# turboderp-org/exllamav2

Measured on NVIDIA H100. Metric: decode tokens/sec (bs=1) Llama2-7B EXL2-4.0bpw, higher is better.
Workload: dtype fp16 (int2-8 weights, fp32 accumulate)

## Files before the change

### exllamav2_b200/csrc/gemv_i8.cu

```cuda
#include <string.h>

#include <algorithm>
#include <map>
#include <mutex>
#include <string>
#include <vector>

#include "gemv_i8.cuh"

namespace exl2b {

constexpr int I8_MAX_WARPS = 16;
constexpr int I8_MAX_CTAS = 320;

struct I8Mat {
    const uint8_t* packed;
    const void* wtab;
    const half* bias;
    half* c;
    half* c_perm;
    const uint16_t* out_invperm;
    int N, blk_base, clear;
};

constexpr uint32_t DF_FLUSH = 1, DF_BLOCK_DONE = 2, DF_GPTQ = 4;
constexpr int I8_BARS = 8;
constexpr int I8_LWIN = 2 * I8_BARS;

struct I8Params {
    I8Mat mat[I8_MAX_MATS];
    const uint4* plan_desc;
    const uint32_t* plan_first;
    const uint32_t* plan_cta;
    const uint32_t* plan_red;
    int num_mats, K, KS;
    const uint16_t* perm;
    const half* x;
    const half* x2;
    const half* norm_w;
    float norm_eps;
    int mode, x_permuted;
    int norm_permuted;
    int l2_prefetch;
    int arena;
    int srow;
    int busy_ctas;
    unsigned int* slot_cnt;
    unsigned long long* dbg;
    int dbg_cta;
    unsigned long long* dbg_rec;
};

struct I8Smem {
    uint32_t act, asum, ascale, emit, scl, lst, total;
};
__host__ __device__ inline I8Smem i8_smem_map(int warps, int arena, int KS, int srow) {
    auto up = [](uint32_t x) { return (x + 15u) & ~15u; };
    I8Smem m;
    m.act = up((uint32_t)warps * (uint32_t)arena);
    m.asum = up(m.act + (uint32_t)KS * 64u);
    m.ascale = up(m.asum + (uint32_t)KS * 4u);
    m.emit = up(m.ascale + (uint32_t)(KS / 4 + 1) * 4u);
    m.scl = up(m.emit + (uint32_t)warps * 256u);
    m.lst = up(m.scl + (uint32_t)(warps * I8_BARS * srow));
    m.total = up(m.lst + (uint32_t)(warps * I8_LWIN * 16));
    return m;
}

template <int BITS>
__device__ __forceinline__ void consume_slab(uint32_t wb, uint32_t xs, int lane, int (&am)[4], int (&ae)[2]) {
    constexpr int Pm = plane_main(BITS), Pe = plane_extra(BITS);
    if constexpr (BITS == 4) {
        const uint4 w4 = lds128(wb + lane * 16);
#pragma unroll
        for (int hf = 0; hf < 2; ++hf) {
            const uint4 xh = lds128(xs + hf * 16), xl = lds128(xs + 32 + hf * 16);
            const uint32_t wa = hf ? w4.z : w4.x, wc = hf ? w4.w : w4.y;
            const uint32_t lo0 = wa & 0x0f0f0f0fu, hi0 = wa & 0xf0f0f0f0u, lo1 = wc & 0x0f0f0f0fu, hi1 = wc & 0xf0f0f0f0u;
            am[0] = dp4a_us(lo0, xh.x, am[0]);
            am[1] = dp4a_uu(lo0, xl.x, am[1]);
            am[2] = dp4a_us(hi0, xh.y, am[2]);
            am[3] = dp4a_uu(hi0, xl.y, am[3]);
            am[0] = dp4a_us(lo1, xh.z, am[0]);
            am[1] = dp4a_uu(lo1, xl.z, am[1]);
            am[2] = dp4a_us(hi1, xh.w, am[2]);
            am[3] = dp4a_uu(hi1, xl.w, am[3]);
        }
        return;
    }
    uint32_t XH[8], XL[8];
    {
        const uint4 h0 = lds128(xs), h1 = lds128(xs + 16), l0 = lds128(xs + 32), l1 = lds128(xs + 48);
        XH[0] = h0.x; XH[1] = h0.y; XH[2] = h0.z; XH[3] = h0.w; XH[4] = h1.x; XH[5] = h1.y; XH[6] = h1.z; XH[7] = h1.w;
        XL[0] = l0.x; XL[1] = l0.y; XL[2] = l0.z; XL[3] = l0.w; XL[4] = l1.x; XL[5] = l1.y; XL[6] = l1.z; XL[7] = l1.w;
    }
    if constexpr (Pm == 4) {
        const uint4 w4 = lds128(wb + lane * 16);
        const uint32_t W[4] = {w4.x, w4.y, w4.z, w4.w};
#pragma unroll
        for (int j = 0; j < 4; ++j) {
            const uint32_t lo = W[j] & 0x0f0f0f0fu, hi = W[j] & 0xf0f0f0f0u;
            am[0] = dp4a_us(lo, XH[2 * j], am[0]);
            am[1] = dp4a_uu(lo, XL[2 * j], am[1]);
            am[2] = dp4a_us(hi, XH[2 * j + 1], am[2]);
            am[3] = dp4a_uu(hi, XL[2 * j + 1], am[3]);
        }
    } else if constexpr (Pm == 8) {
        const uint4 a4 = lds128(wb + lane * 16), b4 = lds128(wb + 512 + lane * 16);
        const uint32_t W[8] = {a4.x, a4.y, a4.z, a4.w, b4.x, b4.y, b4.z, b4.w};
#pragma unroll
        for (int w = 0; w < 8; ++w) {
            am[0] = dp4a_us(W[w], XH[w], am[0]);
            am[1] = dp4a_uu(W[w], XL[w], am[1]);
        }
    } else {
        const uint2 w2 = lds64(wb + lane * 8);
        const uint32_t W[2] = {w2.x, w2.y};
#pragma unroll
        for (int w = 0; w < 2; ++w)
#pragma unroll
            for (int i = 0; i < 4; ++i) {
                const uint32_t t = (W[w] >> (2 * i)) & 0x03030303u;
                am[0] = dp4a_us(t, XH[4 * w + i], am[0]);
                am[1] = dp4a_uu(t, XL[4 * w + i], am[1]);
            }
    }
    if constexpr (Pe == 1) {
        const uint32_t w = lds32(wb + 128 * Pm + lane * 4);
#pragma unroll
        for (int i = 0; i < 8; ++i) {
            const uint32_t t = (w >> i) & 0x01010101u;
            ae[0] = dp4a_us(t, XH[i], ae[0]);
            ae[1] = dp4a_uu(t, XL[i], ae[1]);
        }
    } else if constexpr (Pe == 2) {
        const uint2 w2 = lds64(wb + 128 * Pm + lane * 8);
        const uint32_t W[2] = {w2.x, w2.y};
#pragma unroll
        for (int w = 0; w < 2; ++w)
#pragma unroll
            for (int i = 0; i < 4; ++i) {
                const uint32_t t = (W[w] >> (2 * i)) & 0x03030303u;
                ae[0] = dp4a_us(t, XH[4 * w + i], ae[0]);
                ae[1] = dp4a_uu(t, XL[4 * w + i], ae[1]);
            }
    }
}

template <int BITS>
__device__ __forceinline__ int consume_stage(uint32_t slot, int n, uint32_t xs, uint32_t asum, int lane, int (&am)[4], int (&ae)[2]) {
    constexpr uint32_t bb = 128 * BITS;
    int S = 0;
    if constexpr (BITS == 4) {
        uint4 w4 = lds128(slot + lane * 16);
#pragma unroll 1
        for (int s = 0; s < n; ++s) {
            const uint4 wn = lds128(slot + (s + 1 < n ? s + 1 : s) * bb + lane * 16);
            const uint32_t x = xs + s * 64;
#pragma unroll
            for (int hf = 0; hf < 2; ++hf) {
                const uint4 xh = lds128(x + hf * 16), xl = lds128(x + 32 + hf * 16);
                const uint32_t wa = hf ? w4.z : w4.x, wc = hf ? w4.w : w4.y;
                const uint32_t lo0 = wa & 0x0f0f0f0fu, hi0 = wa & 0xf0f0f0f0u, lo1 = wc & 0x0f0f0f0fu, hi1 = wc & 0xf0f0f0f0u;
                am[0] = dp4a_us(lo0, xh.x, am[0]);
                am[1] = dp4a_uu(lo0, xl.x, am[1]);
                am[2] = dp4a_us(hi0, xh.y, am[2]);
                am[3] = dp4a_uu(hi0, xl.y, am[3]);
                am[0] = dp4a_us(lo1, xh.z, am[0]);
                am[1] = dp4a_uu(lo1, xl.z, am[1]);
                am[2] = dp4a_us(hi1, xh.w, am[2]);
                am[3] = dp4a_uu(hi1, xl.w, am[3]);
            }
            S += (int)lds32(asum + s * 4);
            w4 = wn;
        }
        return S;
    }
#pragma unroll 1
    for (int s = 0; s < n; ++s) {
        consume_slab<BITS>(slot + s * bb, xs + s * 64, lane, am, ae);
        S += (int)lds32(asum + s * 4);
    }
    return S;
}

struct I8OutPre {
    uint32_t add;
    uint32_t kp;
};
__device__ __forceinline__ int mat_of_block(const I8Params& P, int blk) {
    int mi = 0;
#pragma unroll
    for (int i = 1; i < I8_MAX_MATS; ++i)
        if (i < P.num_mats && blk >= P.mat[i].blk_base) mi = i;
    return mi;
}
__device__ __forceinline__ I8OutPre out_pre(const I8Params& P, int blk, int lane) {
    const I8Mat& m = P.mat[mat_of_block(P, blk)];
    const int n = (blk - m.blk_base) * 32 + lane;
    I8OutPre r = {0u, (uint32_t)n};
    if (n < m.N) {
        if (m.bias) r.add = __ldg(reinterpret_cast<const unsigned short*>(m.bias) + n);
        if (!m.clear) r.add |= (uint32_t)__ldcg(reinterpret_cast<const unsigned short*>(m.c) + n) << 16;
        if (m.c_perm && m.out_invperm) r.kp = __ldg(m.out_invperm + n);
    }
    return r;
}
__device__ __forceinline__ void finalize_block(const I8Params& P, int blk, int lane, const I8OutPre& pre, float v) {
    const I8Mat& m = P.mat[mat_of_block(P, blk)];
    const int n = (blk - m.blk_base) * 32 + lane;
    if (n < m.N) {
        v += __half2float(__ushort_as_half((unsigned short)(pre.add & 0xffffu)));
        v += __half2float(__ushort_as_half((unsigned short)(pre.add >> 16)));
        const half h = __float2half_rn(v);
        m.c[n] = h;
        if (m.c_perm) m.c_perm[pre.kp] = h;
    }
}

__device__ __forceinline__ half silu_h(half x) {
    const half e = hexp(__hneg(x));
    const half r = hrcp(__hadd(__float2half(1.0f), e));
    return __hmul(x, r);
}
__device__ __forceinline__ half2 silu_h2(half2 x) {
    const half2 e = h2exp(__hneg2(x));
    const half2 r = h2rcp(__hadd2(__float2half2_rn(1.0f), e));
    return __hmul2(x, r);
}
__device__ __forceinline__ half gelu_h(half x) {
    float xf = __half2float(x);
    const float t = 0.797884560803f * (xf + 0.044715f * xf * xf * xf);
    float th;
    asm("tanh.approx.f32 %0, %1;" : "=f"(th) : "f"(t));
    xf = 0.5f * xf * (1.0 + th);
    return __float2half_rn(xf);
}


template <int I8_WARPS>
__global__ void __launch_bounds__(I8_WARPS * 32, 2) gemv_i8_kernel(const __grid_constant__ I8Params P) {
    constexpr int I8_THREADS = I8_WARPS * 32;
    extern __shared__ __align__(128) uint8_t smem[];
    __shared__ uint64_t bars[I8_WARPS * I8_BARS];
    __shared__ float s_red[I8_WARPS];

    const int tid = threadIdx.x, warp = tid >> 5, lane = tid & 31;
    const int KS = P.KS;
    EXL2B_STAMP(P, 0);
    if (P.dbg_rec && tid == 0 && blockIdx.x < 160) P.dbg_rec[blockIdx.x * 4] = globaltimer();
    if (tid < I8_WARPS * I8_BARS) mbar_init(smem_addr(&bars[tid]), 1);
    mbar_fence_init();
    __syncthreads();
    griddep_launch_dependents();

    if ((int)blockIdx.x >= P.busy_ctas) {
        if (tid == 0) slot_hold(P.slot_cnt, P.busy_ctas);
        return;
    }

    const uint32_t cinfo = __ldg(P.plan_cta + blockIdx.x);
    const int blk0 = (int)(cinfo & 0xffffu), nb = (int)(cinfo >> 16);
    const uint32_t fw0 = __ldg(P.plan_first + blockIdx.x * I8_WARPS + warp), fw1 = __ldg(P.plan_first + blockIdx.x * I8_WARPS + warp + 1);
    const uint32_t f0 = fw0 & 0x3ffffffu, f1 = fw1 & 0x3ffffffu;
    const int nst = (int)(f1 - f0), n_pre = (int)(fw0 >> 26);
    const uint4* const list = P.plan_desc + f0;

    const I8Smem sm = i8_smem_map(I8_WARPS, P.arena, KS, P.srow);
    uint8_t* const act_g = smem + sm.act;
    int* const asum_s = reinterpret_cast<int*>(smem + sm.asum);
    float* const ascale_s = reinterpret_cast<float*>(smem + sm.ascale);
    float* const emit_base = reinterpret_cast<float*>(smem + sm.emit);
    uint32_t sbase;
    asm volatile("mov.u32 %0, %1;" : "=r"(sbase) : "r"(smem_addr(smem)));
    const uint32_t ring = sbase + (uint32_t)warp * (uint32_t)P.arena;
    const uint32_t act = sbase + sm.act, asum = sbase + sm.asum, ascale = sbase + sm.ascale;
    const uint32_t sring = sbase + sm.scl + (uint32_t)(warp * I8_BARS * P.srow), lwin = sbase + sm.lst + (uint32_t)(warp * I8_LWIN * 16);
    uint32_t bar0;
    asm volatile("mov.u32 %0, %1;" : "=r"(bar0) : "r"(smem_addr(&bars[warp * I8_BARS])));

    auto issue_stages = [&](int s0, int cnt, uint4 d) {
        if (lane < cnt) {
            const int s = s0 + lane;
            const uint32_t mi = (d.z >> 22) & 3u;
            const uint8_t* pk = mi == 0 ? P.mat[0].packed : (mi == 1 ? P.mat[1].packed : P.mat[2].packed);
            const uint8_t* wt = reinterpret_cast<const uint8_t*>(mi == 0 ? P.mat[0].wtab : (mi == 1 ? P.mat[1].wtab : P.mat[2].wtab));
            const uint32_t bytes = ((d.z >> 24) & 0xffu) << 7;
            const uint32_t esz = (d.z & (DF_GPTQ << 18)) ? 4u : 2u;
            const uint32_t sbytes = (d.z & (DF_FLUSH << 18)) ? 32u * esz : 0u;
            const bool lnext = s + I8_BARS < nst;
            const uint32_t slot = (uint32_t)s & (I8_BARS - 1);
            const uint32_t bar = bar0 + slot * 8u;
            mbar_arrive_expect_tx(bar, bytes + sbytes + (lnext ? 16u : 0u));
            bulk_copy_g2s(ring + ((d.w >> 16) & 0xffu) * 128u, pk + d.x, bytes, bar);
            if (sbytes) bulk_copy_g2s(sring + slot * (uint32_t)P.srow, wt + (size_t)d.y * esz, sbytes, bar);
            if (lnext) bulk_copy_g2s(lwin + ((uint32_t)(s + I8_BARS) & (I8_LWIN - 1)) * 16u, list + s + I8_BARS, 16u, bar);
        }
    };
    uint4 dfirst = make_uint4(0u, 0u, 0u, 0u);
    if (lane < I8_BARS && lane < nst) {
        dfirst = __ldg(list + lane);
        stu128(lwin + (uint32_t)lane * 16u, dfirst);
    }
    fence_proxy_async();
    __syncwarp();
    EXL2B_STAMP(P, 8);
    issue_stages(0, n_pre, dfirst);
    int next_req = n_pre;
    if (P.l2_prefetch)
        for (int s0 = n_pre; s0 < nst; s0 += 32) {
            const int s = s0 + lane;
            if (s < nst) {
                const uint4 d = __ldg(list + s);
                const uint32_t mi = (d.z >> 22) & 3u;
                const uint8_t* pk = mi == 0 ? P.mat[0].packed : (mi == 1 ? P.mat[1].packed : P.mat[2].packed);
                bulk_prefetch_l2(pk + d.x, ((d.z >> 24) & 0xffu) << 7);
            }
        }
    EXL2B_STAMP(P, 9);

    const int n_oct = P.K >> 3;
    const bool gather_x = P.perm != nullptr && !P.x_permuted;
    constexpr int PF = 3;
    uint4 pv[PF], wv[PF];
#pragma unroll
    for (int r = 0; r < PF; ++r) {
        const int o = r * I8_THREADS + tid;
        pv[r] = make_uint4(0, 0, 0, 0);
        wv[r] = make_uint4(0, 0, 0, 0);
        if (o < n_oct) {
            if (P.perm && (gather_x || !P.norm_permuted)) pv[r] = __ldg(reinterpret_cast<const uint4*>(P.perm + o * 8));
            if (P.mode == I8_RMSNORM) {
                if (P.perm && !P.norm_permuted) {
                    const uint16_t* pi = reinterpret_cast<const uint16_t*>(&pv[r]);
                    uint16_t* wo = reinterpret_cast<uint16_t*>(&wv[r]);
#pragma unroll
                    for (int e = 0; e < 8; ++e) wo[e] = __half_as_ushort(__ldg(P.norm_w + pi[e]));
                } else {
                    wv[r] = __ldg(reinterpret_cast<const uint4*>(P.norm_w + o * 8));
                }
            }
        }
    }

    EXL2B_STAMP(P, 1);
    griddep_wait();
    EXL2B_STAMP(P, 2);
    if (P.dbg_rec && tid == 0 && blockIdx.x < 160) P.dbg_rec[blockIdx.x * 4 + 1] = globaltimer();

    float sumsq = 0.f;
    const bool two_in = (P.mode == I8_SILU_MUL || P.mode == I8_GELU_MUL);
    const bool smem_gather = gather_x && !two_in && n_oct <= PF * I8_THREADS;
    uint4 hg[PF];
    if (smem_gather) {
        for (int o = tid; o < n_oct; o += I8_THREADS)
            reinterpret_cast<uint4*>(act_g)[o] = __ldcg(reinterpret_cast<const uint4*>(P.x + o * 8));
        __syncthreads();
#pragma unroll
        for (int r = 0; r < PF; ++r) {
            const int o = r * I8_THREADS + tid;
            hg[r] = make_uint4(0, 0, 0, 0);
            if (o < n_oct) {
                const uint16_t* pi = reinterpret_cast<const uint16_t*>(&pv[r]);
                uint16_t* ho = reinterpret_cast<uint16_t*>(&hg[r]);
#pragma unroll
                for (int e = 0; e < 8; ++e) ho[e] = reinterpret_cast<const uint16_t*>(act_g)[pi[e]];
            }
        }
        __syncthreads();
    }
    auto stage_round = [&](int o, uint4 pidx, uint4 wreg, bool pre, uint4 hval) {
        const bool valid = o < n_oct;
        float f[8];
#pragma unroll
        for (int e = 0; e < 8; ++e) f[e] = 0.f;
        if (valid) {
            const uint16_t* pi = reinterpret_cast<const uint16_t*>(&pidx);
            half h[8], h2[8];
            const bool two = two_in;
            if (pre) {
                *reinterpret_cast<uint4*>(h) = hval;
            } else if (gather_x) {
#pragma unroll
                for (int e = 0; e < 8; ++e) h[e] = __ldcg(P.x + pi[e]);
                if (two) {
#pragma unroll
                    for (int e = 0; e < 8; ++e) h2[e] = __ldcg(P.x2 + pi[e]);
                }
            } else {
                const uint4 v = __ldcg(reinterpret_cast<const uint4*>(P.x + o * 8));
                *reinterpret_cast<uint4*>(h) = v;
                if (two) *reinterpret_cast<uint4*>(h2) = __ldcg(reinterpret_cast<const uint4*>(P.x2 + o * 8));
            }
            if (P.mode == I8_RMSNORM) {
                const half* wh = reinterpret_cast<const half*>(&wreg);
#pragma unroll
                for (int e = 0; e < 8; ++e) {
                    const float xf = __half2float(h[e]);
                    sumsq = fmaf(xf, xf, sumsq);
                    f[e] = xf * __half2float(wh[e]);
                }
            } else if (P.mode == I8_SILU_MUL) {
#pragma unroll
                for (int e = 0; e < 8; e += 2) {
                    const float2 p = __half22float2(__hmul2(silu_h2(__halves2half2(h[e], h[e + 1])), __halves2half2(h2[e], h2[e + 1])));
                    f[e] = p.x;
                    f[e + 1] = p.y;
                }
            } else if (P.mode == I8_GELU_MUL) {
#pragma unroll
                for (int e = 0; e < 8; ++e) f[e] = __half2float(__hmul(gelu_h(h[e]), h2[e]));
            } else {
#pragma unroll
                for (int e = 0; e < 8; ++e) f[e] = __half2float(h[e]);
            }
        }
        float amax = 0.f;
#pragma unroll
        for (int e = 0; e < 8; ++e) amax = fmaxf(amax, fabsf(f[e]));
#pragma unroll
        for (int s = 1; s < 16; s <<= 1) amax = fmaxf(amax, __shfl_xor_sync(0xffffffffu, amax, s));
        const uint32_t ef = (__float_as_uint(amax * 1.000030518f) >> 23) & 0xffu;
        const float inv = amax > 0.f ? __uint_as_float((268u - ef) << 23) : 0.f;
        uint32_t qb[8], usum = 0u;
#pragma unroll
        for (int e = 0; e < 8; ++e) {
            qb[e] = __float_as_uint(fmaf(f[e], inv, 12582912.f));
            usum += qb[e];
        }
        int sum = (int)(usum - 8u * 0x4B400000u);
        sum += __shfl_xor_sync(0xffffffffu, sum, 1);
        sum += __shfl_xor_sync(0xffffffffu, sum, 2);
        if (valid) {
            auto pack = [&](int i0, int i1, int i2, int i3, uint32_t sel) -> uint32_t {
                return __byte_perm(__byte_perm(qb[i0], qb[i1], sel), __byte_perm(qb[i2], qb[i3], sel), 0x5410u);
            };
            uint2 hw, lw;
            hw.x = pack(0, 4, 1, 5, 0x0051u); hw.y = pack(2, 6, 3, 7, 0x0051u);
            lw.x = pack(0, 4, 1, 5, 0x0040u); lw.y = pack(2, 6, 3, 7, 0x0040u);
            const int si = o >> 2, j = o & 3;
            *reinterpret_cast<uint2*>(act_g + (size_t)si * 64 + j * 8) = hw;
            *reinterpret_cast<uint2*>(act_g + (size_t)si * 64 + 32 + j * 8) = lw;
            if (j == 0) asum_s[si] = sum;
            if ((o & 15) == 0) ascale_s[si >> 2] = amax > 0.f ? __uint_as_float((ef - 14u) << 23) : 0.f;
        }
    };
#pragma unroll
    for (int r = 0; r < PF; ++r)
        if (r * I8_THREADS < n_oct) stage_round(r * I8_THREADS + tid, pv[r], wv[r], smem_gather, hg[r]);
    for (int ob = PF * I8_THREADS; ob < n_oct; ob += I8_THREADS) {
        const int o = ob + tid;
        uint4 pidx = make_uint4(0, 0, 0, 0), wreg = make_uint4(0, 0, 0, 0);
        if (o < n_oct) {
            if (P.perm && (gather_x || !P.norm_permuted)) pidx = __ldg(reinterpret_cast<const uint4*>(P.perm + o * 8));
            if (P.mode == I8_RMSNORM) {
                if (P.perm && !P.norm_permuted) {
                    const uint16_t* pi = reinterpret_cast<const uint16_t*>(&pidx);
                    uint16_t* wo = reinterpret_cast<uint16_t*>(&wreg);
#pragma unroll
                    for (int e = 0; e < 8; ++e) wo[e] = __half_as_ushort(__ldg(P.norm_w + pi[e]));
                } else {
                    wreg = __ldg(reinterpret_cast<const uint4*>(P.norm_w + o * 8));
                }
            }
        }
        stage_round(o, pidx, wreg, false, make_uint4(0, 0, 0, 0));
    }
    if (P.mode == I8_RMSNORM) {
#pragma unroll
        for (int s = 16; s > 0; s >>= 1) sumsq += __shfl_xor_sync(0xffffffffu, sumsq, s);
        if (lane == 0) s_red[warp] = sumsq;
    }
    __syncthreads();
    EXL2B_STAMP(P, 3);
    float rrms = 1.f;
    if (P.mode == I8_RMSNORM) {
        float t = 0.f;
#pragma unroll
        for (int i = 0; i < I8_WARPS; ++i) t += s_red[i];
        rrms = rsqrtf(t * (1.0f / (float)P.K) + P.norm_eps);
    }

    uint32_t red0 = 0u;
    I8OutPre opre0 = {0u, 0u};
    if (warp < nb) {
        red0 = __ldg(P.plan_red + blk0 + warp);
        if (red0 & 0xffffu) opre0 = out_pre(P, blk0 + warp, lane);
    }

    int am[4] = {0, 0, 0, 0}, ae[2] = {0, 0};
    float tot = 0.f;
    int S = 0, blk_slabs = 0, emits = 0;
#pragma unroll 1
    for (int s = 0; s < nst; ++s) {
        const uint4 d = lds128(lwin + ((uint32_t)s & (I8_LWIN - 1)) * 16u);
        const int nreq = (int)((d.w >> 24) & 15u);
        const uint32_t slot8 = (uint32_t)s & (I8_BARS - 1);
        mbar_wait(bar0 + slot8 * 8u, ((uint32_t)s >> 3) & 1u);
        const int ks = (int)(d.z & 0x7ffu), n = (int)((d.z >> 11) & 7u), bits = (int)((d.z >> 14) & 15u);
        const uint32_t slot = ring + ((d.w >> 16) & 0xffu) * 128u;
        const uint32_t xs = act + (uint32_t)ks * 64u, as = asum + (uint32_t)ks * 4u;
        {
            int bsel = bits;
            auto opaque = [&]() { asm volatile("" : "+r"(bsel)); return bsel; };
            if (bsel == 4) S += consume_stage<4>(slot, n, xs, as, lane, am, ae);
            else if (opaque() == 5) S += consume_stage<5>(slot, n, xs, as, lane, am, ae);
            else if (opaque() == 6) S += consume_stage<6>(slot, n, xs, as, lane, am, ae);
            else if (opaque() == 3) S += consume_stage<3>(slot, n, xs, as, lane, am, ae);
            else if (opaque() == 8) S += consume_stage<8>(slot, n, xs, as, lane, am, ae);
            else S += consume_stage<2>(slot, n, xs, as, lane, am, ae);
        }
        uint4 dreq = make_uint4(0u, 0u, 0u, 0u);
        if (lane < nreq) dreq = lds128(lwin + ((uint32_t)(next_req + lane) & (I8_LWIN - 1)) * 16u);
        uint32_t wraw = 0u;
        if (d.z & (DF_FLUSH << 18))
            wraw = (d.z & (DF_GPTQ << 18)) ? lds32(sring + slot8 * (uint32_t)P.srow + (uint32_t)lane * 4u)
                                           : lds_u16(sring + slot8 * (uint32_t)P.srow + (uint32_t)lane * 2u);
        __syncwarp();
        {
            issue_stages(next_req, nreq, dreq);
            next_req += nreq;
        }
        blk_slabs += n;
        if (d.z & (DF_FLUSH << 18)) {
            int v = ((am[0] << 8) + am[1]) + (((am[2] << 8) + am[3]) >> 4) + (((ae[0] << 8) + ae[1]) << plane_main(bits));
            const float ws = __half2float(__ushort_as_half((unsigned short)(wraw & 0xffffu)));
            const int zero = (d.z & (DF_GPTQ << 18)) ? (int)(wraw >> 16) : (1 << (bits - 1));
            v -= zero * S;
            tot = fmaf((float)v, ws * __uint_as_float(lds32(ascale + (uint32_t)(ks >> 2) * 4u)), tot);
            am[0] = am[1] = am[2] = am[3] = 0;
            ae[0] = ae[1] = 0;
            S = 0;
            if (d.z & (DF_BLOCK_DONE << 18)) {
                const int blk = blk0 + (int)(d.w & 0xffffu);
                if (blk_slabs == KS) {
                    finalize_block(P, blk, lane, out_pre(P, blk, lane), tot * rrms);
                } else {
                    if (emits >= 2) __trap();
                    emit_base[(warp * 2 + emits) * 32 + lane] = tot;
                    ++emits;
                }
                tot = 0.f;
                blk_slabs = 0;
            }
        }
    }
    EXL2B_STAMP(P, 4);
    __syncthreads();
    EXL2B_STAMP(P, 5);

    for (int b = warp; b < nb; b += I8_WARPS) {
        const uint32_t rd = (b == warp) ? red0 : __ldg(P.plan_red + blk0 + b);
        uint32_t m = rd & 0xffffu;
        if (m == 0u) continue;
        int w = __ffs(m) - 1;
        float v = emit_base[(w * 2 + (int)((rd >> 16) & 1u)) * 32 + lane];
        for (m &= m - 1u; m; m &= m - 1u) {
            w = __ffs(m) - 1;
            v += emit_base[(w * 2) * 32 + lane];
        }
        finalize_block(P, blk0 + b, lane, (b == warp) ? opre0 : out_pre(P, blk0 + b, lane), v * rrms);
    }
    if (tid == 0) slot_release(P.slot_cnt);
    if (P.dbg && lane == 0) atomicMax(P.dbg + 7, globaltimer());
    if (P.dbg_rec && tid == 0 && blockIdx.x < 160) {
        unsigned smid;
        asm volatile("mov.u32 %0, %%smid;" : "=r"(smid));
        P.dbg_rec[blockIdx.x * 4 + 2] = globaltimer();
        P.dbg_rec[blockIdx.x * 4 + 3] = smid;
    }
}


bool gemv_i8_enabled() {
    static const bool on = [] {
        const char* e = getenv("EXL2B_GEMV");
        return !(e && e[0] == 't');
    }();
    return on;
}

bool gemv_i8_fusable(const QMatrix* const* qs, int nm) {
    if (nm < 1 || nm > I8_MAX_MATS) return false;
    for (int i = 0; i < nm; ++i) {
        if (!qs[i] || qs[i]->v.layout != LAYOUT_TC || qs[i]->v.K != qs[0]->v.K || qs[i]->device != qs[0]->device) return false;
        if ((qs[i]->v.perm == nullptr) != (qs[0]->v.perm == nullptr)) return false;
    }
    if (nm == 1 || !qs[0]->v.perm) return true;
    const int K = qs[0]->v.K;
    std::vector<uint16_t> p0(K), pi(K);
    if (cudaSetDevice(qs[0]->device) != cudaSuccess) return false;
    if (cudaMemcpy(p0.data(), qs[0]->v.perm, (size_t)K * 2, cudaMemcpyDeviceToHost) != cudaSuccess) return false;
    for (int i = 1; i < nm; ++i) {
        if (qs[i]->v.perm == qs[0]->v.perm) continue;
        if (cudaMemcpy(pi.data(), qs[i]->v.perm, (size_t)K * 2, cudaMemcpyDeviceToHost) != cudaSuccess) return false;
        if (p0 != pi) return false;
    }
    return true;
}

void i8_partition_blocks(const std::vector<uint32_t>& bytes, int ctas, unsigned short* out, int* used) {
    const int nb = (int)bytes.size();
    unsigned long long total = 0, biggest = 0;
    for (uint32_t b : bytes) { total += b; biggest = std::max<unsigned long long>(biggest, b); }
    unsigned long long lo = std::max(biggest, (total + ctas - 1) / ctas), hi = total;
    auto fits = [&](unsigned long long cap) {
        int c = 1;
        unsigned long long acc = 0;
        for (uint32_t b : bytes) {
            if (acc + b > cap) { ++c; acc = 0; }
            acc += b;
        }
        return c <= ctas;
    };
    while (lo < hi) {
        const unsigned long long mid = (lo + hi) / 2;
        if (fits(mid)) hi = mid; else lo = mid + 1;
    }
    int c = 0;
    unsigned long long acc = 0;
    out[0] = 0;
    for (int b = 0; b < nb; ++b) {
        if (acc + bytes[b] > lo) { out[++c] = (unsigned short)b; acc = 0; }
        acc += bytes[b];
    }
    out[++c] = (unsigned short)nb;
    *used = c;
}

__global__ void gather_rows_kernel(half* __restrict__ out, const half* __restrict__ w, const uint16_t* __restrict__ perm, int K) {
    const int i = blockIdx.x * blockDim.x + threadIdx.x;
    if (i < K) out[i] = w[perm[i]];
}
int permuted_norm_copy(const QMatrix* q, const half* norm_w, half** out) {
    *out = nullptr;
    half* p = nullptr;
    EXL2B_CUDA(cudaDeviceSynchronize());
    EXL2B_CUDA(cudaMalloc(&p, (size_t)q->v.K * sizeof(half)));
    gather_rows_kernel<<<(q->v.K + 255) / 256, 256>>>(p, norm_w, q->v.perm, q->v.K);
    g_launch_count++;
    cudaError_t e = cudaGetLastError();
    if (e == cudaSuccess) e = cudaDeviceSynchronize();
    if (e != cudaSuccess) {
        cudaFree(p);
        EXL2B_CUDA(e);
    }
    *out = p;
    return 0;
}

struct I8Plan {
    uint4* d_desc = nullptr;
    uint32_t* d_first = nullptr;
    uint32_t* d_cta = nullptr;
    uint32_t* d_red = nullptr;
    int ctas = 0, lcap = 0, arena = 0, srow = 64;
};
struct I8PlanMat {
    int N, KS, is_gptq, num_regions;
    uint32_t blk_stream_bytes;
    QRegion reg[MAX_REGIONS];
};
static std::map<std::string, I8Plan> g_plans[64];
static std::mutex g_plan_mutex;

static void i8_build_lists(const I8PlanMat* mats, int nm, const unsigned short* cta_blk, int C, int warps, int arena,
                           std::vector<uint4>& desc, std::vector<uint32_t>& first, std::vector<uint32_t>& cta, std::vector<uint32_t>& red,
                           int* lcap) {
    const int KS = mats[0].KS;
    int blk_base[I8_MAX_MATS + 1] = {0};
    for (int i = 0; i < nm; ++i) blk_base[i + 1] = blk_base[i] + (mats[i].N + 31) / 32;
    *lcap = 1;
    red.assign(blk_base[nm], 0u);
    for (int c = 0; c < C; ++c) {
        const int blk0 = cta_blk[c], nb = (int)cta_blk[c + 1] - blk0;
        cta.push_back((uint32_t)blk0 | ((uint32_t)nb << 16));
        const long long units = (long long)nb * KS;
        for (int w = 0; w < warps; ++w) {
            first.push_back((uint32_t)desc.size());
            const int l0 = (int)((units * w) / warps), l1 = (int)((units * (w + 1)) / warps);
            int lin = l0;
            while (lin < l1) {
                const int b = lin / KS, ks = lin - b * KS, blk = blk0 + b;
                int mi = 0;
                while (mi + 1 < nm && blk >= blk_base[mi + 1]) ++mi;
                const I8PlanMat& m = mats[mi];
                int r = 0;
                while (r + 1 < m.num_regions && ks >= m.reg[r + 1].ks_begin) ++r;
                const QRegion& rg = m.reg[r];
                const int r_end = (r + 1 < m.num_regions) ? m.reg[r + 1].ks_begin : KS;
                const int rel = ks - rg.ks_begin, g = rel >> rg.spg_log2;
                const int gend = rg.ks_begin + ((g + 1) << rg.spg_log2);
                const int segend = std::min(std::min(gend, (ks | 3) + 1), std::min(r_end, ks + (l1 - lin)));
                const int len = segend - ks, cap = std::max(1, std::min(4, (arena / 2) / (128 * rg.bits)));
                const int pieces = (len + cap - 1) / cap, n = (len + pieces - 1) / pieces;
                uint32_t flags = (ks + n == segend ? DF_FLUSH : 0u) | ((ks + n == KS || lin + n == l1) ? DF_BLOCK_DONE : 0u) | (m.is_gptq ? DF_GPTQ : 0u);
                if (flags & DF_BLOCK_DONE) flags |= DF_FLUSH;
                const int bim = blk - blk_base[mi];
                uint4 d;
                d.x = (uint32_t)bim * m.blk_stream_bytes + rg.off_base + (uint32_t)rel * 128u * (uint32_t)rg.bits;
                d.y = (uint32_t)(rg.group_base + g) * (uint32_t)m.N + (uint32_t)bim * 32u;
                d.z = (uint32_t)ks | ((uint32_t)n << 11) | ((uint32_t)rg.bits << 14) | (flags << 18) | ((uint32_t)mi << 22) |
                      ((uint32_t)(n * rg.bits) << 24);
                d.w = (uint32_t)b;
                desc.push_back(d);
                lin += n;
            }
            {
                int slabs = 0, emits = 0;
                for (size_t s = first.back(); s < desc.size(); ++s) {
                    const uint4& d = desc[s];
                    slabs += (int)((d.z >> 11) & 7u);
                    if (((d.z >> 18) & 15u) & DF_BLOCK_DONE) {
                        if (slabs != KS) {
                            uint32_t& r = red[blk0 + (int)(d.w & 0xffffu)];
                            if ((r & 0xffffu) == 0) r = (uint32_t)emits << 16;
                            r |= 1u << w;
                            ++emits;
                        }
                        slabs = 0;
                    }
                }
            }
            const size_t w0 = first.back(), nst = desc.size() - w0;
            *lcap = std::max(*lcap, (int)nst);
            std::vector<int> dep(nst, -1);
            {
                struct Live { int idx; uint32_t off, size; };
                std::vector<Live> live;
                uint32_t off = 0;
                int last_dep = -1;
                for (size_t s = 0; s < nst; ++s) {
                    const uint4& d = desc[w0 + s];
                    const uint32_t size = ((d.z >> 11) & 7u) * ((d.z >> 14) & 15u) * 128u;
                    if (off + size > (uint32_t)arena) off = 0;
                    auto overlaps = [&](const Live& l) { return l.off < off + size && off < l.off + l.size; };
                    for (;;) {
                        bool hit = false;
                        for (const Live& l : live) hit = hit || overlaps(l);
                        if (!hit && (int)live.size() < I8_BARS) break;
                        last_dep = live.front().idx;
                        live.erase(live.begin());
                    }
                    dep[s] = last_dep;
                    live.push_back(Live{(int)s, off, size});
                    desc[w0 + s].w |= (off / 128u) << 16;
                    off += size;
                }
            }
            int n_pre = 0;
            for (size_t s = 0; s < nst; ++s) {
                if (dep[s] < 0) ++n_pre;
                else desc[w0 + dep[s]].w += 1u << 24;
            }
            first.back() |= (uint32_t)n_pre << 26;
        }
    }
    first.push_back((uint32_t)desc.size());
}

static int i8_plan_host(const I8PlanMat* mats, int nm, int sms, int warps, I8Plan& pl, std::vector<uint4>& desc,
                        std::vector<uint32_t>& first, std::vector<uint32_t>& cta, std::vector<uint32_t>& red) {
    std::vector<uint32_t> blk_bytes;
    for (int i = 0; i < nm; ++i) {
        for (int b = 0; b < (mats[i].N + 31) / 32; ++b) blk_bytes.push_back(mats[i].blk_stream_bytes);
    }
    EXL2B_REQUIRE(blk_bytes.size() < 65535, "too many column blocks (%zu)", blk_bytes.size());
    EXL2B_REQUIRE((long long)blk_bytes.size() * mats[0].KS < (1ll << 30), "problem too large for 32-bit unit arithmetic");
    unsigned short cta_blk[I8_MAX_CTAS + 1];
    i8_partition_blocks(blk_bytes, sms, cta_blk, &pl.ctas);
    static const int smem_budget = [] { const char* e = getenv("EXL2B_I8_SMEM"); return e ? atoi(e) : 111 * 1024; }();
    pl.srow = 64;
    for (int i = 0; i < nm; ++i)
        if (mats[i].is_gptq) pl.srow = 128;
    pl.arena = 8192;
    for (;;) {
        desc.clear(); first.clear(); cta.clear();
        i8_build_lists(mats, nm, cta_blk, pl.ctas, warps, pl.arena, desc, first, cta, red, &pl.lcap);
        if ((int)i8_smem_map(warps, pl.arena, mats[0].KS, pl.srow).total <= smem_budget || pl.arena <= 2048) break;
        pl.arena -= 128;
    }
    EXL2B_REQUIRE(desc.size() < (1u << 26), "too many stages");
    return 0;
}

static int i8_get_plan(int device, const I8PlanMat* mats, int nm, int sms, int warps, I8Plan* out) {
    std::string key((const char*)mats, sizeof(I8PlanMat) * nm);
    const int extra[3] = {nm, sms, warps};
    key.append((const char*)extra, sizeof(extra));
    std::lock_guard<std::mutex> lk(g_plan_mutex);
    auto it = g_plans[device].find(key);
    if (it != g_plans[device].end()) { *out = it->second; return 0; }

    I8Plan pl;
    std::vector<uint4> desc;
    std::vector<uint32_t> first, cta, red;
    const int rc = i8_plan_host(mats, nm, sms, warps, pl, desc, first, cta, red);
    if (rc) return rc;
    EXL2B_CUDA(cudaMalloc(&pl.d_desc, desc.size() * sizeof(uint4) + 16));
    EXL2B_CUDA(cudaMalloc(&pl.d_first, first.size() * 4));
    EXL2B_CUDA(cudaMalloc(&pl.d_cta, cta.size() * 4));
    EXL2B_CUDA(cudaMemcpy(pl.d_desc, desc.data(), desc.size() * sizeof(uint4), cudaMemcpyHostToDevice));
    EXL2B_CUDA(cudaMemcpy(pl.d_first, first.data(), first.size() * 4, cudaMemcpyHostToDevice));
    EXL2B_CUDA(cudaMemcpy(pl.d_cta, cta.data(), cta.size() * 4, cudaMemcpyHostToDevice));
    EXL2B_CUDA(cudaMalloc(&pl.d_red, red.size() * 4 + 4));
    EXL2B_CUDA(cudaMemcpy(pl.d_red, red.data(), red.size() * 4, cudaMemcpyHostToDevice));
    g_plans[device][key] = pl;
    *out = pl;
    return 0;
}

int gemv_i8_launch(int device, cudaStream_t stream, const I8Out* outs, int nm, const I8Input& in) {
    EXL2B_REQUIRE(nm >= 1 && nm <= I8_MAX_MATS, "bad matrix count %d", nm);
    EXL2B_REQUIRE(device >= 0 && device < 64, "bad device %d", device);
    EXL2B_REQUIRE(in.x, "null input row");
    EXL2B_REQUIRE(in.mode != I8_RMSNORM || in.norm_w, "RMSNorm prologue without a weight");
    EXL2B_REQUIRE((in.mode != I8_SILU_MUL && in.mode != I8_GELU_MUL) || in.x2, "act*mul prologue without the second operand");
    static const int warps = [] {
        const char* e = getenv("EXL2B_I8_WARPS");
        const int w = e ? atoi(e) : 16;
        return (w == 12 || w == 8) ? w : 16;
    }();
    static bool attr_set[64] = {false};
    if (!attr_set[device]) {
        EXL2B_CUDA(cudaFuncSetAttribute(gemv_i8_kernel<16>, cudaFuncAttributeMaxDynamicSharedMemorySize, 200 * 1024));
        EXL2B_CUDA(cudaFuncSetAttribute(gemv_i8_kernel<12>, cudaFuncAttributeMaxDynamicSharedMemorySize, 200 * 1024));
        EXL2B_CUDA(cudaFuncSetAttribute(gemv_i8_kernel<8>, cudaFuncAttributeMaxDynamicSharedMemorySize, 200 * 1024));
        attr_set[device] = true;
    }

    I8Params P = {};
    P.num_mats = nm;
    P.K = outs[0].q->v.K;
    P.KS = outs[0].q->v.KS;
    P.perm = outs[0].q->v.perm;
    P.x = in.x;
    P.x2 = in.x2;
    P.norm_w = in.norm_w;
    P.norm_eps = in.norm_eps;
    P.mode = in.mode;
    P.x_permuted = in.x_permuted;
    if (in.mode == I8_RMSNORM && P.perm && in.norm_wp) {
        P.norm_w = in.norm_wp;
        P.norm_permuted = 1;
    }
    I8PlanMat pm[I8_MAX_MATS];
    memset(pm, 0, sizeof(pm));
    int blk = 0;
    for (int i = 0; i < nm; ++i) {
        const QMatrix* q = outs[i].q;
        EXL2B_REQUIRE(q && outs[i].c, "null matrix / output");
        const QMatView& v = q->v;
        EXL2B_REQUIRE(v.layout == LAYOUT_TC, "matrix is not in the default (LAYOUT_TC) layout");
        EXL2B_REQUIRE(v.KS == P.KS, "fused matrices must share K");
        EXL2B_REQUIRE((v.perm == nullptr) == (P.perm == nullptr), "fused matrices must share their row permutation");
        EXL2B_REQUIRE(q->wtab, "matrix has no scale table");
        EXL2B_REQUIRE(v.N % 8 == 0, "width %d is not a multiple of 8", v.N);
        EXL2B_REQUIRE(q->packed_bytes < (1ull << 32), "matrix too large for 32-bit stage offsets");
        I8Mat& m = P.mat[i];
        m.packed = reinterpret_cast<const uint8_t*>(v.packed);
        m.wtab = q->wtab;
        m.bias = v.bias;
        m.c = outs[i].c;
        m.c_perm = outs[i].c_perm;
        m.out_invperm = outs[i].out_invperm;
        m.clear = outs[i].clear;
        m.N = v.N;
        m.blk_base = blk;
        blk += (v.N + 31) / 32;
        pm[i].N = v.N;
        pm[i].KS = v.KS;
        pm[i].is_gptq = v.is_gptq;
        pm[i].num_regions = v.num_regions;
        pm[i].blk_stream_bytes = v.blk_stream_bytes;
        for (int r = 0; r < v.num_regions; ++r) pm[i].reg[r] = v.reg[r];
    }
    EXL2B_REQUIRE(P.KS <= 2048, "K = %d exceeds the stage descriptor (K <= 65536)", P.K);
    I8Plan pl;
    static const int double_mb = [] { const char* e = getenv("EXL2B_I8_DOUBLE_MB"); return e ? atoi(e) : 0; }();
    unsigned long long launch_bytes = 0;
    for (int i = 0; i < nm; ++i) launch_bytes += outs[i].q->packed_bytes;
    const int slots = (double_mb > 0 && launch_bytes >= (unsigned long long)double_mb << 20) ? 2 : 1;
    const int grid_ctas = std::min(device_sm_count(device) * slots, I8_MAX_CTAS);
    int rc = i8_get_plan(device, pm, nm, grid_ctas, warps, &pl);
    if (rc) return rc;
    P.plan_desc = pl.d_desc;
    P.plan_first = pl.d_first;
    P.plan_cta = pl.d_cta;
    P.plan_red = pl.d_red;
    P.arena = pl.arena;
    P.srow = pl.srow;
    P.busy_ctas = pl.ctas;
    static const int l2pf = [] { const char* e = getenv("EXL2B_I8_L2PF"); return e ? atoi(e) : 0; }();
    P.l2_prefetch = l2pf;
    const size_t smem_total = i8_smem_map(warps, P.arena, P.KS, P.srow).total;
    EXL2B_REQUIRE(smem_total <= 200 * 1024, "shared memory budget exceeded (%zu bytes, K = %d)", smem_total, P.K);
    extern unsigned long long* g_dbg;
    extern int g_dbg_cta, g_dbg_slot;
    P.dbg = g_dbg ? g_dbg + 32 * (g_dbg_slot++ % 64) : nullptr;
    P.dbg_cta = g_dbg_cta;
    extern unsigned long long* g_dbg_rec;
    P.dbg_rec = (g_dbg_rec && P.dbg) ? g_dbg_rec + (size_t)((g_dbg_slot - 1) % 64) * 160 * 4 : nullptr;
    static SlotCounters slot_cnts;
    rc = next_slot_counter(slot_cnts, device, &P.slot_cnt);
    if (rc) return rc;
    const int C = slot_holders_disabled() ? pl.ctas : std::max(pl.ctas, grid_ctas);
    if (warps == 16) EXL2B_CUDA(launch_pdl_f("i8", gemv_i8_kernel<16>, dim3(C), dim3(16 * 32), smem_total, stream, P));
    else if (warps == 12) EXL2B_CUDA(launch_pdl_f("i8", gemv_i8_kernel<12>, dim3(C), dim3(12 * 32), smem_total, stream, P));
    else EXL2B_CUDA(launch_pdl_f("i8", gemv_i8_kernel<8>, dim3(C), dim3(8 * 32), smem_total, stream, P));
    return 0;
}

}

extern "C" int exl2b_row_gemv_i8(void) { return exl2b::gemv_i8_enabled() ? 1 : 0; }

extern "C" int exl2b_debug_partition(const uint32_t* block_bytes, int num_blocks, int ctas, uint16_t* out, int* used) {
    EXL2B_REQUIRE(block_bytes && out && used && num_blocks > 0 && ctas > 0 && ctas <= exl2b::I8_MAX_CTAS, "bad argument");
    std::vector<uint32_t> b(block_bytes, block_bytes + num_blocks);
    exl2b::i8_partition_blocks(b, ctas, out, used);
    return 0;
}

extern "C" int exl2b_debug_plan(int N, int KS, int is_gptq, uint32_t blk_stream_bytes, const int* regions, int num_regions, int ctas, int warps,
                                int slot_bytes, uint32_t* desc, int cap_desc, uint32_t* first, int* ctas_used, int* n_desc, int* lcap,
                                uint32_t* red) {
    EXL2B_REQUIRE(regions && desc && first && ctas_used && n_desc && lcap, "null argument");
    EXL2B_REQUIRE(num_regions >= 1 && num_regions <= exl2b::MAX_REGIONS && ctas > 0 && ctas <= exl2b::I8_MAX_CTAS && warps > 0, "bad argument");
    exl2b::I8PlanMat m;
    memset(&m, 0, sizeof(m));
    m.N = N; m.KS = KS; m.is_gptq = is_gptq; m.num_regions = num_regions; m.blk_stream_bytes = blk_stream_bytes;
    for (int r = 0; r < num_regions; ++r)
        m.reg[r] = exl2b::QRegion{regions[5 * r], regions[5 * r + 1], regions[5 * r + 2], regions[5 * r + 3], (uint32_t)regions[5 * r + 4]};
    std::vector<uint32_t> bb((N + 31) / 32, blk_stream_bytes);
    unsigned short cta_blk[exl2b::I8_MAX_CTAS + 1];
    exl2b::i8_partition_blocks(bb, ctas, cta_blk, ctas_used);
    std::vector<uint4> d;
    std::vector<uint32_t> f, c, r;
    exl2b::i8_build_lists(&m, 1, cta_blk, *ctas_used, warps, slot_bytes, d, f, c, r, lcap);
    EXL2B_REQUIRE((int)d.size() <= cap_desc, "descriptor buffer too small (%zu)", d.size());
    memcpy(desc, d.data(), d.size() * sizeof(uint4));
    memcpy(first, f.data(), f.size() * 4);
    if (red) memcpy(red, r.data(), r.size() * 4);
    *n_desc = (int)d.size();
    return 0;
}

extern "C" int exl2b_debug_i8_plan(const int* mats, int nm, int ctas, int warps, uint32_t* desc, int cap_desc, uint32_t* first,
                                   int cap_first, int* info) {
    EXL2B_REQUIRE(mats && desc && first && info, "null argument");
    EXL2B_REQUIRE(nm >= 1 && nm <= exl2b::I8_MAX_MATS && ctas > 0 && ctas <= exl2b::I8_MAX_CTAS && warps > 0, "bad argument");
    exl2b::I8PlanMat pm[exl2b::I8_MAX_MATS];
    memset(pm, 0, sizeof(pm));
    for (int i = 0; i < nm; ++i) {
        const int* r = mats + i * (5 + 5 * exl2b::MAX_REGIONS);
        EXL2B_REQUIRE(r[4] >= 1 && r[4] <= exl2b::MAX_REGIONS && r[1] == mats[1], "bad matrix %d", i);
        pm[i].N = r[0]; pm[i].KS = r[1]; pm[i].is_gptq = r[2]; pm[i].blk_stream_bytes = (uint32_t)r[3]; pm[i].num_regions = r[4];
        for (int g = 0; g < r[4]; ++g) {
            const int* q = r + 5 + 5 * g;
            pm[i].reg[g] = exl2b::QRegion{q[0], q[1], q[2], q[3], (uint32_t)q[4]};
        }
    }
    exl2b::I8Plan pl;
    std::vector<uint4> d;
    std::vector<uint32_t> f, c, red;
    const int rc = exl2b::i8_plan_host(pm, nm, ctas, warps, pl, d, f, c, red);
    if (rc) return rc;
    EXL2B_REQUIRE((int)d.size() <= cap_desc && (int)f.size() <= cap_first, "output buffers too small (%zu, %zu)", d.size(), f.size());
    memcpy(desc, d.data(), d.size() * sizeof(uint4));
    memcpy(first, f.data(), f.size() * 4);
    info[0] = pl.ctas;
    info[1] = (int)d.size();
    info[2] = pl.arena;
    info[3] = pl.srow;
    info[4] = (int)exl2b::i8_smem_map(warps, pl.arena, pm[0].KS, pl.srow).total;
    info[5] = pl.lcap;
    return 0;
}
```

Measured before the change: 489.7.

## Rebalance GEMV work split, enable budgeted L2 prefetch, hoist activation loads

Makes the L2 prefetch of upcoming weight stages on by default, limited to a per-warp byte budget computed with a warp prefix sum. Activation loads are hoisted ahead of the compute rounds so they overlap the weight fetch. The host planner now splits blocks across CTAs by even byte shares rather than greedy packing, and splits units across warps by cumulative byte cost rather than unit count. Together these aim to cut load imbalance and memory latency stalls, at the cost of more register pressure, extra L2 traffic and more host-side planning work.

```diff
diff --git a/exllamav2_b200/csrc/gemv_i8.cu b/exllamav2_b200/csrc/gemv_i8.cu
--- a/exllamav2_b200/csrc/gemv_i8.cu
+++ b/exllamav2_b200/csrc/gemv_i8.cu
@@ -41,7 +41,7 @@
     float norm_eps;
     int mode, x_permuted;
     int norm_permuted;
-    int l2_prefetch;
+    int l2_budget;
     int arena;
     int srow;
     int busy_ctas;
@@ -307,16 +307,23 @@
     EXL2B_STAMP(P, 8);
     issue_stages(0, n_pre, dfirst);
     int next_req = n_pre;
-    if (P.l2_prefetch)
-        for (int s0 = n_pre; s0 < nst; s0 += 32) {
-            const int s = s0 + lane;
-            if (s < nst) {
-                const uint4 d = __ldg(list + s);
-                const uint32_t mi = (d.z >> 22) & 3u;
-                const uint8_t* pk = mi == 0 ? P.mat[0].packed : (mi == 1 ? P.mat[1].packed : P.mat[2].packed);
-                bulk_prefetch_l2(pk + d.x, ((d.z >> 24) & 0xffu) << 7);
-            }
-        }
+    if (P.l2_budget > 0) {
+        const int s = n_pre + lane;
+        uint4 d = make_uint4(0u, 0u, 0u, 0u);
+        if (s < nst) d = __ldg(list + s);
+        const uint32_t bytes = ((d.z >> 24) & 0xffu) << 7;
+        uint32_t past = bytes;
+#pragma unroll
+        for (int o = 1; o < 32; o <<= 1) {
+            const uint32_t t = __shfl_up_sync(0xffffffffu, past, o);
+            if (lane >= o) past += t;
+        }
+        if (s < nst && past - bytes < (uint32_t)P.l2_budget) {
+            const uint32_t mi = (d.z >> 22) & 3u;
+            const uint8_t* pk = mi == 0 ? P.mat[0].packed : (mi == 1 ? P.mat[1].packed : P.mat[2].packed);
+            bulk_prefetch_l2(pk + d.x, bytes);
+        }
+    }
     EXL2B_STAMP(P, 9);
 
     const int n_oct = P.K >> 3;
@@ -351,49 +358,64 @@
     float sumsq = 0.f;
     const bool two_in = (P.mode == I8_SILU_MUL || P.mode == I8_GELU_MUL);
     const bool smem_gather = gather_x && !two_in && n_oct <= PF * I8_THREADS;
-    uint4 hg[PF];
+    auto load_round = [&](int o, uint4 pidx, uint4& h, uint4& h2) {
+        if (o >= n_oct) return;
+        if (gather_x) {
+            const uint16_t* pi = reinterpret_cast<const uint16_t*>(&pidx);
+            uint16_t* ho = reinterpret_cast<uint16_t*>(&h);
+            uint16_t* ho2 = reinterpret_cast<uint16_t*>(&h2);
+#pragma unroll
+            for (int e = 0; e < 8; ++e) ho[e] = __ldcg(reinterpret_cast<const unsigned short*>(P.x) + pi[e]);
+            if (two_in) {
+#pragma unroll
+                for (int e = 0; e < 8; ++e) ho2[e] = __ldcg(reinterpret_cast<const unsigned short*>(P.x2) + pi[e]);
+            }
+        } else {
+            h = __ldcg(reinterpret_cast<const uint4*>(P.x + o * 8));
+            if (two_in) h2 = __ldcg(reinterpret_cast<const uint4*>(P.x2 + o * 8));
+        }
+    };
+    uint4 xv[PF];
     if (smem_gather) {
-        for (int o = tid; o < n_oct; o += I8_THREADS)
-            reinterpret_cast<uint4*>(act_g)[o] = __ldcg(reinterpret_cast<const uint4*>(P.x + o * 8));
-        __syncthreads();
 #pragma unroll
         for (int r = 0; r < PF; ++r) {
             const int o = r * I8_THREADS + tid;
-            hg[r] = make_uint4(0, 0, 0, 0);
+            xv[r] = make_uint4(0, 0, 0, 0);
+            if (o < n_oct) xv[r] = __ldcg(reinterpret_cast<const uint4*>(P.x + o * 8));
+        }
+#pragma unroll
+        for (int r = 0; r < PF; ++r)
+            if (r * I8_THREADS + tid < n_oct) reinterpret_cast<uint4*>(act_g)[r * I8_THREADS + tid] = xv[r];
+        __syncthreads();
+#pragma unroll
+        for (int r = 0; r < PF; ++r) {
+            const int o = r * I8_THREADS + tid;
             if (o < n_oct) {
                 const uint16_t* pi = reinterpret_cast<const uint16_t*>(&pv[r]);
-                uint16_t* ho = reinterpret_cast<uint16_t*>(&hg[r]);
+                uint16_t* ho = reinterpret_cast<uint16_t*>(&xv[r]);
 #pragma unroll
                 for (int e = 0; e < 8; ++e) ho[e] = reinterpret_cast<const uint16_t*>(act_g)[pi[e]];
             }
         }
         __syncthreads();
-    }
-    auto stage_round = [&](int o, uint4 pidx, uint4 wreg, bool pre, uint4 hval) {
+    } else {
+#pragma unroll
+        for (int r = 0; r < PF; ++r) {
+            xv[r] = make_uint4(0, 0, 0, 0);
+            load_round(r * I8_THREADS + tid, pv[r], xv[r], wv[r]);
+        }
+    }
+    auto stage_round = [&](int o, uint4 hval, uint4 sval) {
         const bool valid = o < n_oct;
         float f[8];
 #pragma unroll
         for (int e = 0; e < 8; ++e) f[e] = 0.f;
         if (valid) {
-            const uint16_t* pi = reinterpret_cast<const uint16_t*>(&pidx);
             half h[8], h2[8];
-            const bool two = two_in;
-            if (pre) {
-                *reinterpret_cast<uint4*>(h) = hval;
-            } else if (gather_x) {
-#pragma unroll
-                for (int e = 0; e < 8; ++e) h[e] = __ldcg(P.x + pi[e]);
-                if (two) {
-#pragma unroll
-                    for (int e = 0; e < 8; ++e) h2[e] = __ldcg(P.x2 + pi[e]);
-                }
-            } else {
-                const uint4 v = __ldcg(reinterpret_cast<const uint4*>(P.x + o * 8));
-                *reinterpret_cast<uint4*>(h) = v;
-                if (two) *reinterpret_cast<uint4*>(h2) = __ldcg(reinterpret_cast<const uint4*>(P.x2 + o * 8));
-            }
+            *reinterpret_cast<uint4*>(h) = hval;
+            *reinterpret_cast<uint4*>(h2) = sval;
             if (P.mode == I8_RMSNORM) {
-                const half* wh = reinterpret_cast<const half*>(&wreg);
+                const half* wh = h2;
 #pragma unroll
                 for (int e = 0; e < 8; ++e) {
                     const float xf = __half2float(h[e]);
@@ -447,10 +469,10 @@
     };
 #pragma unroll
     for (int r = 0; r < PF; ++r)
-        if (r * I8_THREADS < n_oct) stage_round(r * I8_THREADS + tid, pv[r], wv[r], smem_gather, hg[r]);
+        if (r * I8_THREADS < n_oct) stage_round(r * I8_THREADS + tid, xv[r], wv[r]);
     for (int ob = PF * I8_THREADS; ob < n_oct; ob += I8_THREADS) {
         const int o = ob + tid;
-        uint4 pidx = make_uint4(0, 0, 0, 0), wreg = make_uint4(0, 0, 0, 0);
+        uint4 pidx = make_uint4(0, 0, 0, 0), wreg = make_uint4(0, 0, 0, 0), hval = make_uint4(0, 0, 0, 0);
         if (o < n_oct) {
             if (P.perm && (gather_x || !P.norm_permuted)) pidx = __ldg(reinterpret_cast<const uint4*>(P.perm + o * 8));
             if (P.mode == I8_RMSNORM) {
@@ -464,7 +486,8 @@
                 }
             }
         }
-        stage_round(o, pidx, wreg, false, make_uint4(0, 0, 0, 0));
+        load_round(o, pidx, hval, wreg);
+        stage_round(o, hval, wreg);
     }
     if (P.mode == I8_RMSNORM) {
 #pragma unroll
@@ -546,6 +569,7 @@
         }
     }
     EXL2B_STAMP(P, 4);
+    if (P.dbg && blockIdx.x == P.dbg_cta && lane == 0) P.dbg[10 + warp] = globaltimer();
     __syncthreads();
     EXL2B_STAMP(P, 5);
 
@@ -617,14 +641,29 @@
         const unsigned long long mid = (lo + hi) / 2;
         if (fits(mid)) hi = mid; else lo = mid + 1;
     }
-    int c = 0;
-    unsigned long long acc = 0;
+    auto ctas_from = [&](int b) {
+        int c = 0;
+        unsigned long long acc = 0;
+        for (; b < nb; ++b) {
+            if (c == 0 || acc + bytes[b] > lo) { ++c; acc = 0; }
+            acc += bytes[b];
+        }
+        return c;
+    };
+    int c = 0, b = 0;
+    unsigned long long left = total;
     out[0] = 0;
-    for (int b = 0; b < nb; ++b) {
-        if (acc + bytes[b] > lo) { out[++c] = (unsigned short)b; acc = 0; }
-        acc += bytes[b];
-    }
-    out[++c] = (unsigned short)nb;
+    while (b < nb) {
+        const int rest = ctas - c - 1;
+        const double share = (double)left / (double)(ctas - c);
+        unsigned long long acc = bytes[b++];
+        while (b < nb && acc + bytes[b] <= lo) {
+            if ((double)acc + 0.5 * (double)bytes[b] > share && ctas_from(b) <= rest) break;
+            acc += bytes[b++];
+        }
+        out[++c] = (unsigned short)b;
+        left -= acc;
+    }
     *used = c;
 }
 
@@ -672,13 +711,37 @@
     for (int i = 0; i < nm; ++i) blk_base[i + 1] = blk_base[i] + (mats[i].N + 31) / 32;
     *lcap = 1;
     red.assign(blk_base[nm], 0u);
+    std::vector<unsigned long long> cum;
+    std::vector<int> bound;
     for (int c = 0; c < C; ++c) {
         const int blk0 = cta_blk[c], nb = (int)cta_blk[c + 1] - blk0;
         cta.push_back((uint32_t)blk0 | ((uint32_t)nb << 16));
         const long long units = (long long)nb * KS;
+        cum.assign((size_t)units + 1, 0ull);
+        for (long long u = 0; u < units; ++u) {
+            const int blk = blk0 + (int)(u / KS), ks = (int)(u % KS);
+            int mi = 0;
+            while (mi + 1 < nm && blk >= blk_base[mi + 1]) ++mi;
+            const I8PlanMat& m = mats[mi];
+            int r = 0;
+            while (r + 1 < m.num_regions && ks >= m.reg[r + 1].ks_begin) ++r;
+            const QRegion& rg = m.reg[r];
+            const int r_end = (r + 1 < m.num_regions) ? m.reg[r + 1].ks_begin : KS;
+            const int gend = rg.ks_begin + ((((ks - rg.ks_begin) >> rg.spg_log2) + 1) << rg.spg_log2);
+            const bool flush = ks + 1 == std::min(std::min(gend, (ks | 3) + 1), r_end);
+            cum[u + 1] = cum[u] + 128ull * (unsigned)rg.bits + (flush ? (m.is_gptq ? 128ull : 64ull) : 0ull);
+        }
+        bound.assign(warps + 1, 0);
+        bound[warps] = (int)units;
+        for (int w = 1; w < warps; ++w) {
+            const unsigned long long target = cum[units] * (unsigned long long)w / (unsigned long long)warps;
+            int u = (int)(std::lower_bound(cum.begin(), cum.end(), target) - cum.begin());
+            if (u > 0 && target - cum[u - 1] < cum[u] - target) --u;
+            bound[w] = std::max(bound[w - 1], u);
+        }
         for (int w = 0; w < warps; ++w) {
             first.push_back((uint32_t)desc.size());
-            const int l0 = (int)((units * w) / warps), l1 = (int)((units * (w + 1)) / warps);
+            const int l0 = bound[w], l1 = bound[w + 1];
             int lin = l0;
             while (lin < l1) {
                 const int b = lin / KS, ks = lin - b * KS, blk = blk0 + b;
@@ -891,8 +954,8 @@
     P.arena = pl.arena;
     P.srow = pl.srow;
     P.busy_ctas = pl.ctas;
-    static const int l2pf = [] { const char* e = getenv("EXL2B_I8_L2PF"); return e ? atoi(e) : 0; }();
-    P.l2_prefetch = l2pf;
+    static const int l2pf = [] { const char* e = getenv("EXL2B_I8_L2PF"); return e ? std::max(0, atoi(e)) : 1024; }();
+    P.l2_budget = l2pf;
     const size_t smem_total = i8_smem_map(warps, P.arena, P.KS, P.srow).total;
     EXL2B_REQUIRE(smem_total <= 200 * 1024, "shared memory budget exceeded (%zu bytes, K = %d)", smem_total, P.K);
     extern unsigned long long* g_dbg;
```

Result: faster. 502.0 (median of 6 runs) (+2.5%).
